# Leo-Liao-Chao/Uncertainty-Aware-CILQR-for-Trajectory-Optimization

Measured on AMD Instinct MI355X. Metric: CILQR solves/sec (N=50, batch B), higher is better.
Workload: dtype f64

## Files before the change

### uncertainty-aware-cilqr-for-trajectory-optimization_amd/csrc/cilqr_solve.hip

```cpp
#include <type_traits>

#include "cilqr_device.hpp"

namespace cilqr {

using namespace dev;

namespace {

constexpr int FREC = 16;

__device__ __forceinline__ double readfirstlane_f64(double v) {
  int lo = __double2loint(v), hi = __double2hiint(v);
  lo = __builtin_amdgcn_readfirstlane(lo);
  hi = __builtin_amdgcn_readfirstlane(hi);
  return __hiloint2double(hi, lo);
}

__device__ __forceinline__ double wave_sum(double v) {
#pragma unroll
  for (int o = 32; o > 0; o >>= 1) v += __shfl_xor(v, o, WAVE);
  return v;
}

// ... 414 lines not shown
  mfma_place(cur.AA, cur.sAA, slotA, low, cst);
  mfma_place(cur.BB, cur.sBB, slotB, low, cst);
  mfma_place(cur.Ca, cur.sCa, odd ? slotX : slotXX, low, cst);
  mfma_place(cur.Cb, cur.sCb, odd ? slotUU : C0, low, cst);
  double m00 = e == 0 ? 1.0 : 0.0, m01 = e == 1 || e == 4 ? 1.0 : 0.0, m11 = e == 5 ? 1.0 : 0.0;
  double mvc = odd && (lane & 3) == 2 ? 1.0 : 0.0;
  double lamb = lamb_in, lamb0 = lamb_in * (inv_half_dt * inv_half_dt);
  double lamb_row = (lane >> 4) == 0 ? lamb0 : lamb;
  CILQR_PIN(m00); CILQR_PIN(m01); CILQR_PIN(m11); CILQR_PIN(mvc); CILQR_PIN(lamb); CILQR_PIN(lamb0); CILQR_PIN(lamb_row);
  const bool stores = lane == 6 || lane == 22 || lane < 4 || (lane >= 16 && lane < 20);
  const int gslot = lane == 6 ? 0 : lane == 22 ? 1 : lane < 4 ? 2 + lane : 6 + (lane & 3);
  unsigned goff = stores ? (unsigned)(((N - 1) * FREC + gslot) * 8) : (unsigned)((N * FREC + (lane & 15)) * 8);
  const unsigned gstride = stores ? FREC * 8 : 0;
  char* const gbase = reinterpret_cast<char*>(fwd);
  double* gp = kK + (N - 1) * RECF + (stores ? gslot : 10 + (lane & 3));

  MfmaOperands oa, ob;
  cur.upper(oa);
  double V = odd_blocks_from_even(oa.Ca), vc = oa.Ca * mvc;
  int signs_v = 0, signs_s = 0;
  double det0 = 0.0;
  auto step = [&](const MfmaOperands& o) {
    unsigned long long s0 = 0, s1 = 0, s2 = 0, s3 = 0;
    if (DIAG) stamp_request(s0, V);
    const double P = CILQR_MFMA(V, o.AB, vc);
    const double Db = CILQR_MFMA(o.BB, P, o.Cb);
    const double Da = CILQR_MFMA(o.AA, P, o.Ca);
    const double a = readlane_f64(Db, 4), b = readlane_f64(Db, 5), d = readlane_f64(Db, 21);
    if (DIAG) stamp_request(s1, a + b + d);
    const double bb = b * b;
    det0 = fma(a, d, -bb);
    signs_v |= __double2hiint(det0);
    signs_s |= __double2hiint(a) | __double2hiint(d);
    const double ar = a + lamb0, dr = d + lamb;
    const double nr = -rcp_newton(fma(ar, dr, -bb));
    if (DIAG) stamp_request(s2, nr);
    const double adj = fma(ar, m11, fma(-b, m01, dr * m00));
    const double Dk = CILQR_MFMA(adj, Db, 0.0) * nr;
    const double H0 = fma(lamb_row, Dk, Db);
    const double H = odd_blocks_from_even(H0);
    double Dv = CILQR_MFMA(H, Dk, Da);
    vc = Dv * mvc;
    CILQR_PIN(vc);
    CILQR_PIN(Dv);
    V = odd_blocks_from_even(Dv);
    if (FSMEM) {
      *reinterpret_cast<double*>(gbase + goff) = Dk;
      goff -= gstride;
      asm volatile("" : "+v"(goff));
    } else {
      *gp = Dk;
      gp -= RECF;
    }
    if (DIAG) {
      stamp_request(s3, V);
      stamps_collect(s0, s1, s2, s3);
      sub[5] += s1 - s0; sub[6] += s2 - s1; sub[7] += s3 - s2;
    }
  };
  auto trip = [&] {
    cur.lower(ob);
    step(oa);
    cur.back();
    cur.upper(oa);
    step(ob);
  };
  bool two_left;
  if (FSMEM) {
    two_left = ((N - 1) & 1) != 0;
    for (int trips = (N - 1) >> 1; trips > 0; --trips) trip();
  } else {
    int j = N - 1;
    for (; j >= 2; j -= 2) trip();
    two_left = j == 1;
  }
  if (two_left) {
    cur.lower(ob);
    step(oa);
    step(ob);
  } else {
    step(oa);
  }
  return __builtin_amdgcn_ballot_w64((signs_v | signs_s) < 0 || !(det0 == det0)) == 0;
}

template <int KS>
__device__ __forceinline__ void load_fwd(FwdIn& o, const double* X, const double* U, const double* kK, int i) {
  const double* xo = X + i * XR;
  o.x = xo[0]; o.y = xo[1]; o.v = xo[2]; o.th = xo[3];
  o.u0 = U[2 * i]; o.u1 = U[2 * i + 1];
  const double* g = kK + i * KS;
#pragma unroll
  for (int k = 0; k < KR; ++k) o.g[k] = g[k];
}

__device__ __forceinline__ void fwd_step_store(const FwdConst& k, const FwdIn& c, State& s, double& max_turn, double inv_half_dt,
                                               double* Un_i, double* Xn_next) {
  double u0, u1;
  forward_step<true>(k, c, s, max_turn, u0, u1, inv_half_dt);
  Un_i[0] = u0; Un_i[1] = u1;
  Xn_next[0] = s.x; Xn_next[1] = s.y; Xn_next[2] = s.v; Xn_next[3] = s.th; Xn_next[4] = s.c; Xn_next[5] = s.s;
}

typedef double d2_t __attribute__((ext_vector_type(2)));
typedef __attribute__((address_space(3))) d2_t lds_d2;
constexpr int FSTEP = FREC * 8;
static_assert(XR % 2 == 0, "state records are whole 16-byte pairs");
struct FwdBump {
  unsigned& off;
  lds_d2*& un;
  lds_d2*& xn;
  template <int J> __device__ __forceinline__ void pin(double& ps, double& pc) const {
    if (J == 0) {
      asm volatile("" : "+v"(ps), "+v"(pc) : "v"(un));
      un += 2;
      asm volatile("" : "+v"(un));
    } else if (J == 1) {
      asm volatile("" : "+v"(ps), "+v"(pc) : "v"(xn));
      xn += XR;
      asm volatile("" : "+v"(xn));
    } else if (J == 2) {
      asm volatile("" : "+v"(ps), "+v"(pc) : "s"(off));
      off += 2 * FSTEP;
      asm volatile("" : "+s"(off));
    } else {
      CILQR_PIN2(ps, pc);
    }
  }
};
typedef double d8_t __attribute__((ext_vector_type(8)));
struct FwdS { d8_t lo, hi; };
__device__ __forceinline__ void f_sload_first(FwdS& r, const double* p) {
  asm volatile("s_load_dwordx16 %0, %2, 0x0\n\ts_load_dwordx16 %1, %2, 0x40" : "=&s"(r.lo), "=&s"(r.hi) : "s"(p) : "memory");
}
template <int AHEAD>
__device__ __forceinline__ void f_sload_next(FwdS& r, const double* fwd, unsigned off) {
  asm volatile("s_load_dwordx16 %0, %2, %3 offset:%4\n\ts_load_dwordx16 %1, %2, %3 offset:%5"
               : "+s"(r.lo), "+s"(r.hi) : "s"(fwd), "s"(off), "n"(AHEAD), "n"(AHEAD + 64) : "memory");
}
__device__ __forceinline__ void f_swait(FwdS& r) {
  __builtin_amdgcn_s_waitcnt(0xC07F);
  asm volatile("" : "+s"(r.lo), "+s"(r.hi) : : "memory");
}
__device__ __forceinline__ void f_sunpack(FwdIn& o, const FwdS& r) {
  o.g[0] = r.lo[0]; o.g[1] = r.lo[1]; o.g[2] = r.lo[2]; o.g[3] = r.lo[3]; o.g[4] = r.lo[4]; o.g[5] = r.lo[5];
  o.g[6] = r.lo[6]; o.g[7] = r.lo[7]; o.g[8] = r.hi[0]; o.g[9] = r.hi[1];
  o.x = r.hi[2]; o.y = r.hi[3]; o.v = r.hi[4]; o.th = r.hi[5]; o.u0 = r.hi[6]; o.u1 = r.hi[7];
}

template <bool PUBLISH = false>
__device__ __forceinline__ bool forward_smem(const KParams& kp, int N, const double* X, const double* fwd, double* Xn, double* Un) {
  asm volatile("s_waitcnt vmcnt(0)\n\ts_dcache_inv\n\ts_waitcnt lgkmcnt(0)" ::: "memory");
  FwdConst k;
  make_fwd_const(k, kp);
  double ihd = 2.0 / kp.dt;
  CILQR_PIN(ihd);
  State s;
  s.x = X[0]; s.y = X[1]; s.v = X[2]; s.th = X[3]; s.c = X[4]; s.s = X[5];
  store_state(Xn, 0, s);
  double max_turn = 0.0;
  FwdS r;
  FwdIn c;
  f_sload_first(r, fwd);
  unsigned off = 0;
  lds_d2* un = (lds_d2*)Un;
  lds_d2* xn = (lds_d2*)(Xn + XR);
// ... 149 lines not shown

  const double* wts = TAB != 2 ? obs_weights(a, b) : nullptr;
  if (TAB == 2) {
    sampled_prologue<WAVE>(a, kp, b, N, M, tab, off, rmax);
  } else if (!tab_shared) {
    const bool held = a.obs_ts == 0;
    for (int m = 0; m < M; ++m) {
      ObsEntry e;
      if (held) e = obs_entry_at(kp, a, b, m, 0);
      for (int t = lane; t < N; t += WAVE) {
        if (!held) e = obs_entry_at(kp, a, b, m, t);
        double* o = tab + ((size_t)m * N + t) * TABF;
        o[0] = e.ox; o[1] = e.oy; o[2] = e.co; o[3] = e.so; o[4] = e.ia2; o[5] = e.ib2;
      }
    }
  }
  __syncthreads();
  {
    double m = 0.0;
    for (int q = lane; q + 1 < S; q += WAVE) {
      const double d = fabs(samp[q + 1] - samp[q]);
      m = fmax(m, d == d ? d : __builtin_huge_val());
    }
    grid.dmax = wave_max_uniform(m);
  }

  UncPose upose{0, 0, 1, 0};
  if (has_unc) upose = unc_pose(a.unc, b);
  bool handover = false;
  if (GENERAL) {
    const double* x0 = a.x0 + (size_t)b * 4;
    State s;
    s.x = x0[0]; s.y = x0[1]; s.v = x0[2]; s.th = x0[3];
    sincos_fast(s.th, &s.s, &s.c);
    if (lane == 0) store_state(Xa, 0, s);
    for (int i = 0; i < N; ++i) {
      s = dyn_step(kp, s, Ua[2 * i], Ua[2 * i + 1]);
      if (lane == 0) store_state(Xa, i + 1, s);
    }
  } else {
    handover = !rollout_fast(kp, N, a.x0 + (size_t)b * 4, Ua, Xa) || (a.flags & CILQR_FLAG_GENERAL_ONLY) != 0;
  }
  __syncthreads();

  CILQR_STAMP(c_pro)
  double* Xc = Xa;
  double* Uc = Ua;
  double* Xn = Xb;
  double* Un = Ub;
  double J_old = DBL_MAX, lamb = 1.0, J_new = 0.0;
  int iters = 0, status = CILQR_EXIT_MAX_ITER, n_pass = 0;
  bool j_valid = false;
  const bool faithful = (a.flags & CILQR_FLAG_FAITHFUL_ITERS) != 0;
  const int max_it = kp.max_iterations;
  for (int it = 0; it < max_it && !handover; ++it) {
    ++iters;
    {
      double part;
      const KParams kpl = phase_params();
      const UncArgs* unc = has_unc ? &phase_args().unc : nullptr;
      if (TAB == 2) part = linearize<RECW, FSMEM, DIAG>(kpl, N, n_entries, lane, samp, S, grid, Xc, Uc, rec, SampledSource{tab, off, rmax, Xc, N, a.n_samples, M, a.samp_w, kpl.ego_front, kpl.ego_rear,
                                                     sqrt(1.0 + 64.0 / kpl.q2_front), sqrt(1.0 + 64.0 / kpl.q2_rear)}, unc, upose, b, fwd, sub);
      else part = linearize<RECW, FSMEM, DIAG>(kpl, N, n_entries, lane, samp, S, grid, Xc, Uc, rec, TabSource<TAB == 0>{tab, wts, N, kpl.w_obstacle}, unc, upose, b, fwd, sub);
      unsigned long long sub_t = 0;
      if (DIAG) sub_t = stamp_after(part);
      J_new = wave_sum_uniform(part);
      CILQR_SUB(4, J_new)
    }
    j_valid = true;
    __syncthreads();
    CILQR_STAMP(c_L)
    if (DIAG) ++n_L;
    const bool accept = J_new < J_old;
    if (!accept && !faithful) {
      if (J_new != J_new) { status = CILQR_EXIT_NUMERIC; break; }
      for (;;) {
        lamb = lamb * kp.lamb_factor;
        if (lamb > kp.lamb_max) { status = CILQR_EXIT_LAMBDA_MAX; break; }
        if (++it >= max_it) { status = CILQR_EXIT_MAX_ITER; break; }
        ++iters;
      }
      break;
    }
    if (!(GENERAL ? riccati<true>(kp, N, rec, kK, lamb) : riccati_mfma<FSMEM, DIAG>(N, rec, kK, fwd, cst, 2.0 / kp.dt, lamb, sub))) {
      if (GENERAL) { status = CILQR_EXIT_NUMERIC; break; }
      handover = true;
      break;
    }
    __syncthreads();
    CILQR_STAMP(c_R)
    ++n_pass;
    if (DIAG) ++n_R;
    if (GENERAL) {
      forward_general(kp, N, Xc, Uc, kK, Xn, Un);
    } else if (!(FSMEM ? forward_smem(KParams(phase_params()), N, Xc, fwd, Xn, Un) : forward_fast<RECW>(KParams(phase_params()), N, Xc, Uc, kK, Xn, Un))) {
      handover = true;
      break;
    }
    __syncthreads();
    CILQR_STAMP(c_F)
    if (accept) {
      double* t0 = Xc; Xc = Xn; Xn = t0;
      double* t1 = Uc; Uc = Un; Un = t1;
      j_valid = false;
      lamb = lamb / kp.lamb_factor;
      if (fabs(J_new - J_old) < kp.tolerance) { status = CILQR_EXIT_TOLERANCE; break; }
    } else {
      lamb = lamb * kp.lamb_factor;
      if (lamb > kp.lamb_max) { status = CILQR_EXIT_LAMBDA_MAX; break; }
    }
    J_old = J_new;
  }

  if (!GENERAL) {
    int32_t* const hint = phase_args().hint_passes;
    if (lane == 0) {
      phase_args().redo[b] = handover ? 1 : 0;
      if (handover && hint) hint[b] = 63;
    }
    if (handover) return;
  }

  __syncthreads();
  const SolveArgs ae = phase_args();
  double* Uo = ae.U + (size_t)b * 2 * N;
  for (int i = lane; i < 2 * N; i += WAVE) Uo[i] = Uc[i];
  double* Xg = ae.X_out + (size_t)b * 4 * (N + 1);
  for (int i = lane; i < 4 * (N + 1); i += WAVE) Xg[i] = Xc[(i >> 2) * XR + (i & 3)];
  if (ae.J_out) {
    if (!j_valid) J_new = wave_sum_uniform(cost_only(ae.kp, N, lane, samp, S, grid, Xc, Uc));
    if (lane == 0) ae.J_out[b] = J_new;
  }
  if (lane == 0) {
    if (ae.iters_out) ae.iters_out[b] = iters;
    if (ae.status_out) ae.status_out[b] = status;
    if (ae.passes) ae.passes[b] = n_pass;
    if (ae.hint_passes && !GENERAL) ae.hint_passes[b] = n_pass;
  }
  if (DIAG && lane == 0 && a.diag) {
    const unsigned long long now_ = __builtin_readcyclecounter();
    unsigned long long* o = a.diag + (size_t)b * DIAG_SLOTS;
    o[0] = c_pro; o[1] = c_L; o[2] = c_R; o[3] = c_F; o[4] = now_ - tk; o[5] = n_L; o[6] = n_R; o[7] = now_ - tk0;
    for (int q = 0; q < 8; ++q) o[8 + q] = sub[q];
  }
#undef CILQR_STAMP
}

constexpr unsigned long long THETA_PENDING = 0x7FF00000DEADBEEFull;
constexpr int PAIR_SPIN = 1 << 16;
constexpr int CMD_GO = 1, CMD_EXIT = 2;
constexpr int PAIR_LAST = 10;

template <int K>
__device__ __forceinline__ double quad_bcast(double v) {
  return dpp_f64<K * 0x55>(v);
}
template <int K>
__device__ __forceinline__ int quad_bcast_i(int v) { return __builtin_amdgcn_update_dpp(v, v, K * 0x55, 0xF, 0xF, false); }

template <bool LONG_NAP>
__device__ __forceinline__ bool state_arrived(const double* X, int k, int& budget) {
  const volatile unsigned long long* p = reinterpret_cast<const volatile unsigned long long*>(X + k * XR + 3);
  while (*p == THETA_PENDING) {
    if (--budget < 0) return false;
    if (LONG_NAP) __builtin_amdgcn_s_sleep(16); else __builtin_amdgcn_s_sleep(1);
  }
  asm volatile("" ::: "memory");
// ... 149 lines not shown
  double* Xa = samp + ((S + 1) & ~1);
  double* Ua = Xa + (N + 1) * XR;
  double* rec = Ua + 2 * N;
  double* cst = rec + N * RECF;
  double* tab = cst + RCST;
  double* Jt = tab + (size_t)M * TABF * N;
  double* ctl = Jt + ((N + 1) & ~1);
  double* fwd = a.fwd + (size_t)b * (N + 1) * FREC;
  int* const cmd = reinterpret_cast<int*>(ctl + 1);

  SampleGrid grid;
  make_sample_grid(grid, a.xplan_fl[2 * b], a.xplan_fl[2 * b + 1], S);
  {
    const double* pc = a.poly + (size_t)b * CILQR_POLY_COEFFS;
    for (int s = tid; s < S; s += 2 * WAVE) {
      double xs;
      sample_xy(grid, pc, s, xs, samp[s]);
    }
  }
  const double* Ug = a.U + (size_t)b * 2 * N;
  for (int i = tid; i < 2 * N; i += 2 * WAVE) Ua[i] = Ug[i];
  if (tid < 16 && (tid & 7) < 5) cst[(tid & 7) + (tid >> 3) * RECF] = (tid & 7) == 0 ? 0.0 : (tid & 7) == 1 ? 1.0 : (tid & 7) == 2 ? kp.dt : (tid & 7) == 3 ? kp.w_vel * 2 : 2.0;
  const double* wts = obs_weights(a, b);
  for (int m = wave; m < M; m += 2) {
    for (int t = lane; t < N; t += WAVE) {
      const ObsEntry e = obs_entry_at(kp, a, b, m, t);
      double* o = tab + ((size_t)m * N + t) * TABF;
      o[0] = e.ox; o[1] = e.oy; o[2] = e.co; o[3] = e.so; o[4] = e.ia2; o[5] = e.ib2;
    }
  }
  mark_pending(Xa, N, tid, 2 * WAVE);
  if (tid == 0) { cmd[0] = 0; cmd[1] = 0; }
  __syncthreads();

  if (wave != 0) {
    {
      double m = 0.0;
      for (int q = lane; q + 1 < S; q += WAVE) {
        const double d = fabs(samp[q + 1] - samp[q]);
        m = fmax(m, d == d ? d : __builtin_huge_val());
      }
      grid.dmax = wave_max_uniform(m);
    }
    unsigned long long dg[4] = {0, 0, 0, 0};
    for (;;) {
      linearize_quads<DIAG>(KParams(phase_params()), N, M, lane, samp, S, grid, Xa, Ua, rec, tab, wts, fwd, Jt, ctl, dg);
      __syncthreads();
      __syncthreads();
      if (*reinterpret_cast<volatile int*>(cmd) != CMD_GO) break;
    }
    if (DIAG && lane == 0 && a.diag) {
      unsigned long long* o = a.diag + (size_t)b * DIAG_SLOTS + 8;
      o[0] = dg[0]; o[1] = dg[1]; o[2] = dg[2]; o[3] = dg[3];
    }
    return;
  }

  bool handover = !rollout_fast<true>(kp, N, a.x0 + (size_t)b * 4, Ua, Xa) || (a.flags & CILQR_FLAG_GENERAL_ONLY) != 0;
  const int dbg = DIAG ? (int)((a.flags >> 8) & 3) : 0;
  if (dbg) __syncthreads();
  __syncthreads();
  CILQR_STAMP(c_pro)
  double J_old = DBL_MAX, lamb = 1.0, J_new = 0.0;
  int iters = 0, status = CILQR_EXIT_MAX_ITER, n_pass = 0;
  const int max_it = kp.max_iterations;
  for (int it = 0; it < max_it && !handover; ++it) {
    ++iters;
    if (reinterpret_cast<volatile int*>(cmd)[1] != 0) { handover = true; break; }
    J_new = *reinterpret_cast<volatile double*>(ctl);
    if (DIAG) ++n_L;
    const bool accept = J_new < J_old;
    if (!accept) {
      if (J_new != J_new) { status = CILQR_EXIT_NUMERIC; break; }
      for (;;) {
        lamb = lamb * kp.lamb_factor;
        if (lamb > kp.lamb_max) { status = CILQR_EXIT_LAMBDA_MAX; break; }
        if (++it >= max_it) { status = CILQR_EXIT_MAX_ITER; break; }
        ++iters;
      }
      break;
    }
    mark_pending(Xa, N, lane, WAVE);
    CILQR_STAMP(c_L)
    if (!riccati_mfma<true, DIAG>(N, rec, rec, fwd, cst, 2.0 / kp.dt, lamb, sub)) { handover = true; break; }
    if (lane == 0) *reinterpret_cast<volatile int*>(cmd) = CMD_GO;
    __syncthreads();
    CILQR_STAMP(c_R)
    ++n_pass;
    if (DIAG) ++n_R;
    const bool f_ok = forward_smem<true>(KParams(phase_params()), N, Xa, fwd, Xa, Ua);
    CILQR_STAMP(c_F)
    if (dbg) __syncthreads();
    __syncthreads();
    CILQR_STAMP(c_L)
    if (!f_ok) { handover = true; break; }
    lamb = lamb / kp.lamb_factor;
    if (fabs(J_new - J_old) < kp.tolerance) {
      status = CILQR_EXIT_TOLERANCE;
      J_new = *reinterpret_cast<volatile double*>(ctl);
      break;
    }
    J_old = J_new;
    if (it + 1 >= max_it) J_new = *reinterpret_cast<volatile double*>(ctl);
  }
  if (lane == 0) *reinterpret_cast<volatile int*>(cmd) = CMD_EXIT;
  __syncthreads();

  int32_t* const hint = phase_args().hint_passes;
  if (lane == 0) {
    phase_args().redo[b] = handover ? 1 : 0;
    if (handover && hint) hint[b] = 63;
  }
  if (handover) return;

  const SolveArgs ae = phase_args();
  double* Uo = ae.U + (size_t)b * 2 * N;
  for (int i = lane; i < 2 * N; i += WAVE) Uo[i] = Ua[i];
  double* Xg = ae.X_out + (size_t)b * 4 * (N + 1);
  for (int i = lane; i < 4 * (N + 1); i += WAVE) Xg[i] = Xa[(i >> 2) * XR + (i & 3)];
  if (lane == 0) {
    if (ae.J_out) ae.J_out[b] = J_new;
    if (ae.iters_out) ae.iters_out[b] = iters;
    if (ae.status_out) ae.status_out[b] = status;
    if (ae.passes) ae.passes[b] = n_pass;
    if (ae.hint_passes) ae.hint_passes[b] = n_pass;
  }
  if (DIAG && lane == 0 && a.diag) {
    const unsigned long long now_ = __builtin_readcyclecounter();
    unsigned long long* o = a.diag + (size_t)b * DIAG_SLOTS;
    o[0] = c_pro; o[1] = c_L; o[2] = c_R; o[3] = c_F; o[4] = now_ - tk; o[5] = n_L; o[6] = n_R; o[7] = now_ - tk0;
    for (int q = 4; q < 8; ++q) o[8 + q] = sub[q];
  }
#undef CILQR_STAMP
}

template <int W, bool DIAG, bool UNC = false>
__global__ __launch_bounds__(W * WAVE, 2) void cilqr_solve_split_kernel(SolveArgs a) {
  unsigned long long tk0 = 0, tk = 0, c_pro = 0, c_L = 0, c_R = 0, c_F = 0, n_L = 0, n_R = 0;
  if (DIAG) tk0 = tk = __builtin_readcyclecounter();
#define CILQR_STAMP(acc)                                 \
  if (DIAG) {                                            \
    const unsigned long long now_ = __builtin_readcyclecounter(); \
    acc += now_ - tk;                                    \
    tk = now_;                                           \
  }
  extern __shared__ __attribute__((aligned(16))) double lds[];
  if ((int)blockIdx.x >= a.B) return;
  const int b = __builtin_amdgcn_readfirstlane(a.order ? a.order[blockIdx.x] : (int)blockIdx.x);
  if (b >= a.B) return;
  const int tid = threadIdx.x, lane = tid & (WAVE - 1);
  const int wave = __builtin_amdgcn_readfirstlane(tid >> 6);
  const KParams kp = a.kp;
  const int N = a.N, M = a.M, S = kp.n_samples, NSMP = a.n_samples;
  double* samp = lds;
  double* Xa = samp + ((S + 1) & ~1);
  double* Ua = Xa + (N + 1) * XR;
  double* rec = Ua + 2 * N;
  double* cst = rec + N * RECF;
  double* off = cst + RCST;
  double* rmax = off + (size_t)M * NSMP * OFFF;
  double* part = rmax + 2 * M;
  double* umap = part + (size_t)(W - 1) * 5 * N;
  double* ctl = part + ((((W - 1) + (UNC ? 1 : 0)) * 5 * N + 1) & ~1);
  int* const cmd = reinterpret_cast<int*>(ctl);
  double* tab = a.obs_tab + (size_t)b * M * NOMF * N;

  SampleGrid grid;
// ... 334 lines not shown
  for (int it = 0; it < max_it && !handover; ++it) {
    ++iters;
    {
      const KParams kpl = phase_params();
      double dx[STEPS], dy[STEPS], lx2[STEPS], Jt = 0.0;
#pragma unroll
      for (int c2 = 0; c2 < STEPS; ++c2) {
        dx[c2] = 0.0; dy[c2] = 0.0; lx2[c2] = 0.0;
        const int t = lane + c2 * WAVE;
        if (t < N) {
          const double* xr = Xa + t * XR;
          const double px = xr[0], py = xr[1], v = xr[2];
          const double u0 = Ua[2 * t], u1 = Ua[2 * t + 1];
          double2* q = reinterpret_cast<double2*>(fwd + t * FREC + 10);
          q[0] = make_double2(px, py);
          q[1] = make_double2(v, xr[3]);
          q[2] = make_double2(u0, u1);
          const int cs = closest_sample(S, grid, px, py, LdsSamples{samp, grid.xf, grid.dxs});
          dx[c2] = px - fma(grid.dxs, (double)cs, grid.xf);
          dy[c2] = py - samp[cs];
          const double dv = v - kpl.desired_speed;
          lx2[c2] = (2 * kpl.w_vel) * dv;
          Jt += stage_cost(kpl, dx[c2], dy[c2], dv, u0, u1);
          if (W == 2) {
            Rec c;
            double a1, a2, a3, a4;
            ctrl_args(kpl, u0, u1, v, a1, a2, a3, a4);
            const double e1 = exp_fast(a1);
            const double e2 = exp_fast(a2);
            const double e3 = exp_fast(a3);
            const double e4 = exp_fast(a4);
            ctrl_terms(kpl, u0, u1, e1, e2, e3, e4, c);
            double* r = rec + t * RECF;
            const double ih = 2.0 / kpl.dt;
            r[6] = c.lu0 * ih; r[7] = c.lu1; r[8] = c.luu0 * (ih * ih); r[9] = c.luu1;
          }
        }
      }
      J_new = wave_sum_uniform(Jt);
      unsigned long long w0 = 0;
      if (DIAG) w0 = stamp_after(J_new);
      __syncthreads();
      if (DIAG) c_wait += __builtin_readcyclecounter() - w0;
#pragma unroll
      for (int c2 = 0; c2 < STEPS; ++c2) {
        const int t = lane + c2 * WAVE;
        if (t < N) {
          const double* q = part + (size_t)t * 5;
          StepSums s5{q[0], q[1], q[2], q[3], q[4]};
          if (W == 3 && !UNC) {
            const double* qo = q + (size_t)N * 5;
            s5.lx0 += qo[0]; s5.lx1 += qo[1]; s5.h00 += qo[2]; s5.h01 += qo[3]; s5.h11 += qo[4];
          }
          double* r = rec + t * RECF;
          double lx0, lx1, l00, l01, l11;
          state_terms(kpl, dx[c2], dy[c2], s5, lx0, lx1, l00, l01, l11);
          if (UNC) {
            const double* qu = umap + (size_t)t * 5;
            lx0 += qu[0]; lx1 += qu[1]; l00 += qu[2]; l01 += qu[3]; l11 += qu[4];
          }
          r[0] = lx0; r[1] = lx1; r[2] = lx2[c2]; r[3] = l00; r[4] = l01; r[5] = l11;
        }
      }
      j_valid = true;
    }
    CILQR_STAMP(c_L)
    if (DIAG) ++n_L;
    const bool accept = J_new < J_old;
    bool stop = false;
    if (!accept) {
      if (J_new != J_new) {
        status = CILQR_EXIT_NUMERIC;
      } else {
        for (;;) {
          lamb = lamb * kp.lamb_factor;
          if (lamb > kp.lamb_max) { status = CILQR_EXIT_LAMBDA_MAX; break; }
          if (++it >= max_it) { status = CILQR_EXIT_MAX_ITER; break; }
          ++iters;
        }
      }
      stop = true;
    } else {
      asm volatile("s_waitcnt lgkmcnt(0)" ::: "memory");
      if (!riccati_mfma<true, false>(N, rec, rec, fwd, cst, 2.0 / kp.dt, lamb, nullptr)) {
        handover = true;
        stop = true;
      } else {
        CILQR_STAMP(c_R)
        ++n_pass;
        if (DIAG) ++n_R;
        if (!forward_smem(KParams(phase_params()), N, Xa, fwd, Xa, Ua)) {
          handover = true;
          stop = true;
        } else {
          j_valid = false;
          lamb = lamb / kp.lamb_factor;
          if (fabs(J_new - J_old) < kp.tolerance) { status = CILQR_EXIT_TOLERANCE; stop = true; }
          J_old = J_new;
          if (it + 1 >= max_it) stop = true;
        }
      }
    }
    if (stop && lane == 0) *reinterpret_cast<volatile int*>(cmd) = CMD_EXIT;
    __syncthreads();
    CILQR_STAMP(c_F)
    if (stop) break;
  }

  int32_t* const hint = phase_args().hint_passes;
  if (lane == 0) {
    phase_args().redo[b] = handover ? 1 : 0;
    if (handover && hint) hint[b] = 63;
  }
  if (handover) return;

  const SolveArgs ae = phase_args();
  double* Uo = ae.U + (size_t)b * 2 * N;
  for (int i = lane; i < 2 * N; i += WAVE) Uo[i] = Ua[i];
  double* Xg = ae.X_out + (size_t)b * 4 * (N + 1);
  for (int i = lane; i < 4 * (N + 1); i += WAVE) Xg[i] = Xa[(i >> 2) * XR + (i & 3)];
  if (ae.J_out) {
    if (!j_valid) J_new = wave_sum_uniform(cost_only(ae.kp, N, lane, samp, S, grid, Xa, Ua));
    if (lane == 0) ae.J_out[b] = J_new;
  }
  if (lane == 0) {
    if (ae.iters_out) ae.iters_out[b] = iters;
    if (ae.status_out) ae.status_out[b] = status;
    if (ae.passes) ae.passes[b] = n_pass;
    if (ae.hint_passes) ae.hint_passes[b] = n_pass;
  }
  if (DIAG && lane == 0 && a.diag) {
    const unsigned long long now_ = __builtin_readcyclecounter();
    unsigned long long* o = a.diag + (size_t)b * DIAG_SLOTS;
    o[0] = c_pro; o[1] = c_L; o[2] = c_R; o[3] = c_F; o[4] = now_ - tk; o[5] = n_L; o[6] = n_R; o[7] = now_ - tk0;
    o[10] = c_wait;
    o[12] = (unsigned long long)__builtin_amdgcn_s_getreg((4) | (0 << 6) | (31 << 11)) |
            ((unsigned long long)__builtin_amdgcn_s_getreg((20) | (0 << 6) | (31 << 11)) << 32);
    if (W == 2) { o[11] = 0; o[14] = 0; }
    o[15] = 0;
  }
#undef CILQR_STAMP
}

__global__ void quu_inverse_kernel(int n, const double* q, const double* lamb, double* out, int general) {
  const int i = blockIdx.x * blockDim.x + threadIdx.x;
  if (i >= n) return;
  const double a = q[4 * i], b = 0.5 * (q[4 * i + 1] + q[4 * i + 2]), d = q[4 * i + 3];
  double i00 = 0, i01 = 0, i11 = 0;
  bool ok = true;
  if (general) ok = quu_inverse_general(a, b, d, lamb[i], i00, i01, i11);
  else quu_inverse_psd(a, b, d, lamb[i], b * b, i00, i01, i11);
  const double nan = __builtin_nan("");
  out[4 * i] = ok ? i00 : nan; out[4 * i + 1] = ok ? i01 : nan; out[4 * i + 2] = ok ? i01 : nan; out[4 * i + 3] = ok ? i11 : nan;
}

__global__ void closest_sample_kernel(int n, int S, const double* in, int32_t* out) {
  const int i = blockIdx.x * blockDim.x + threadIdx.x;
  if (i >= n) return;
  const double* q = in + (size_t)i * 10;
  double pc[CILQR_POLY_COEFFS];
  for (int j = 0; j < CILQR_POLY_COEFFS; ++j) pc[j] = q[j];
  SampleGrid g;
  make_sample_grid(g, q[6], q[7], S);
  auto at = [&](int s, double& x, double& y) { sample_xy(g, pc, s, x, y); };
  double m = 0.0, A = 0.0, B = 0.0, yp = 0.0;
  for (int s = 0; s < S; ++s) {
    double x, y, a2, a3;
// ... 130 lines not shown
```

Measured before the change: 2.498 million.

## Add LDS-addressed MFMA Riccati backward pass with deferred PSD check

Adds a specialized Riccati backward pass for the shared-memory path. It reads operands through explicit LDS address-space pointers with per-lane slot cursors. The positive-definiteness and NaN check is moved out of the serial recursion into a parallel post-pass over the stored Q blocks, which removes per-step sign tracking from the critical path. It also writes Q blocks back to LDS and gains into fwd inside the loop. Call sites in the FSMEM and persistent paths now use it, except the W==3 variant, trading more code and extra LDS writes for a shorter dependency chain.

```diff
diff --git a/uncertainty-aware-cilqr-for-trajectory-optimization_amd/csrc/cilqr_solve.hip b/uncertainty-aware-cilqr-for-trajectory-optimization_amd/csrc/cilqr_solve.hip
--- a/uncertainty-aware-cilqr-for-trajectory-optimization_amd/csrc/cilqr_solve.hip
+++ b/uncertainty-aware-cilqr-for-trajectory-optimization_amd/csrc/cilqr_solve.hip
@@ -520,6 +520,141 @@
     step(oa);
   }
   return __builtin_amdgcn_ballot_w64((signs_v | signs_s) < 0 || !(det0 == det0)) == 0;
+}
+
+typedef __attribute__((address_space(3))) double lds_f64;
+struct MfmaLdsCursor {
+  const lds_f64 *AB, *AA, *BB, *Ca, *Cb;
+  int sAB, sAA, sBB, sCa, sCb;
+  __device__ __forceinline__ void upper(MfmaOperands& o) const { o.AB = AB[RECF]; o.AA = AA[RECF]; o.BB = BB[RECF]; o.Ca = Ca[RECF]; o.Cb = Cb[RECF]; }
+  __device__ __forceinline__ void lower(MfmaOperands& o) const { o.AB = AB[0]; o.AA = AA[0]; o.BB = BB[0]; o.Ca = Ca[0]; o.Cb = Cb[0]; }
+};
+__device__ __forceinline__ void mfma_place(const lds_f64*& ptr, int& stride, int slot, const lds_f64* low, const lds_f64* cst) {
+  ptr = slot >= 0 ? low + slot : cst + (-1 - slot);
+  stride = slot >= 0 ? 2 * RECF : 0;
+}
+
+template <bool DIAG>
+__device__ __forceinline__ bool riccati_mfma_smem(int N, const double* rec, double* fwd, const double* cst, double inv_half_dt, double lamb_in,
+                                                  unsigned long long* sub) {
+  constexpr int C0 = -1, C1 = -2, CDT = -3, CW = -4, C2 = -5;
+  const int lane = threadIdx.x;
+  const int e = ((lane >> 4) << 2) | (lane & 3);
+  const bool odd = (lane & 4) != 0;
+  const int slotA = e == 0 || e == 5 || e == 10 || e == 15 ? C1 : e == 2 ? 10 : e == 6 ? 11 : e == 3 ? 12 : e == 7 ? 13 : C0;
+  const int slotB = e == 0 ? 10 : e == 4 ? 11 : e == 8 ? C2 : e == 13 ? CDT : C0;
+  const int slotXX = e == 0 ? 3 : e == 1 || e == 4 ? 4 : e == 5 ? 5 : e == 10 ? CW : C0;
+  const int slotX = e == 2 ? 0 : e == 6 ? 1 : e == 10 ? 2 : C0;
+  const int slotUU = e == 0 ? 8 : e == 5 ? 9 : e == 2 ? 6 : e == 6 ? 7 : C0;
+  using PTR = const lds_f64*;
+  const PTR low = (PTR)rec + (N - 2) * RECF;
+  const PTR cstp = (PTR)cst;
+  MfmaLdsCursor cur;
+  mfma_place(cur.AB, cur.sAB, odd ? slotB : slotA, low, cstp);
+  mfma_place(cur.AA, cur.sAA, slotA, low, cstp);
+  mfma_place(cur.BB, cur.sBB, slotB, low, cstp);
+  mfma_place(cur.Ca, cur.sCa, odd ? slotX : slotXX, low, cstp);
+  mfma_place(cur.Cb, cur.sCb, odd ? slotUU : C0, low, cstp);
+  double m00 = e == 0 ? 1.0 : 0.0, m01 = e == 1 || e == 4 ? 1.0 : 0.0, m11 = e == 5 ? 1.0 : 0.0;
+  double mvc = odd && (lane & 3) == 2 ? 1.0 : 0.0;
+  double lamb = lamb_in, lamb0 = lamb_in * (inv_half_dt * inv_half_dt);
+  double lamb_row = (lane >> 4) == 0 ? lamb0 : lamb;
+  CILQR_PIN(m00); CILQR_PIN(m01); CILQR_PIN(m11); CILQR_PIN(mvc); CILQR_PIN(lamb); CILQR_PIN(lamb0); CILQR_PIN(lamb_row);
+  const bool stores = lane == 6 || lane == 22 || lane < 4 || (lane >= 16 && lane < 20);
+  const int gslot = lane == 6 ? 0 : lane == 22 ? 1 : lane < 4 ? 2 + lane : 6 + (lane & 3);
+  unsigned goff = stores ? (unsigned)(((N - 1) * FREC + gslot) * 8) : (unsigned)((N * FREC + (lane & 15)) * 8);
+  const unsigned gstride = stores ? FREC * 8 : 0;
+  char* const gbase = reinterpret_cast<char*>(fwd);
+  lds_f64* qp = (lds_f64*)rec + (N - 2) * RECF + (lane == 4 ? 0 : lane == 5 ? 1 : lane == 21 ? 2 : 3 + lane % 11);
+
+  MfmaOperands oa, ob;
+  cur.upper(oa);
+  double V = odd_blocks_from_even(oa.Ca), vc = oa.Ca * mvc;
+  auto step = [&](const MfmaOperands& o, auto kind, auto upper_step) {
+    constexpr int KIND = decltype(kind)::value, QOFF = decltype(upper_step)::value ? RECF : 0;
+    unsigned long long s0 = 0, s1 = 0, s2 = 0, s3 = 0;
+    if (DIAG) stamp_request(s0, V);
+    const double P = CILQR_MFMA(V, o.AB, vc);
+    double Db = CILQR_MFMA(o.BB, P, o.Cb);
+    const double Da = CILQR_MFMA(o.AA, P, o.Ca);
+    if (KIND != 3) {
+      asm volatile("" : "+v"(Db) : "v"(cur.AB), "v"(cur.AA), "v"(cur.BB), "v"(cur.Ca), "v"(cur.Cb));
+      if (KIND == 1) cur.upper(oa); else cur.lower(ob);
+      asm volatile("");
+    }
+    const double a = readlane_f64(Db, 4), b = readlane_f64(Db, 5), d = readlane_f64(Db, 21);
+    if (DIAG) stamp_request(s1, a + b + d);
+    const double bb = b * b;
+    const double ar = a + lamb0, dr = d + lamb;
+    const double den = fma(ar, dr, -bb);
+    const double adj = fma(ar, m11, fma(-b, m01, dr * m00));
+    double Dkr = CILQR_MFMA(adj, Db, 0.0);
+    double r = __builtin_amdgcn_rcp(den);
+    asm volatile("" : "+v"(Dkr), "+v"(r), "+v"(goff) : "v"(qp));
+    qp[QOFF] = Db;
+    asm volatile("");
+    r = fma(fma(-den, r, 1.0), r, r);
+    r = fma(fma(-den, r, 1.0), r, r);
+    const double nr = -r;
+    if (DIAG) stamp_request(s2, nr);
+    const double Dk = Dkr * nr;
+    double H0 = fma(lamb_row, Dk, Db);
+    if (KIND == 0) {
+      asm volatile("" : "+v"(H0) : "v"(cur.AB), "v"(cur.AA));
+      cur.AB -= cur.sAB; cur.AA -= cur.sAA;
+    }
+    if (KIND == 1) {
+      asm volatile("" : "+v"(H0) : "v"(qp));
+      qp -= 2 * RECF;
+    }
+    double H = odd_blocks_from_even(H0);
+    if (KIND == 0) {
+      asm volatile("" : "+v"(H) : "v"(cur.BB), "v"(cur.Ca));
+      cur.BB -= cur.sBB; cur.Ca -= cur.sCa;
+    }
+    double Dv = CILQR_MFMA(H, Dk, Da);
+    asm volatile("" : "+v"(Dv) : "v"(goff));
+    *reinterpret_cast<double*>(gbase + goff) = Dk;
+    asm volatile("" : "+v"(Dv) : : "memory");
+    vc = Dv * mvc;
+    CILQR_PIN(vc);
+    asm volatile("" : "+v"(Dv) : "v"(goff), "v"(cur.Cb));
+    goff -= gstride;
+    if (KIND == 0) cur.Cb -= cur.sCb;
+    V = odd_blocks_from_even(Dv);
+    if (DIAG) {
+      stamp_request(s3, V);
+      stamps_collect(s0, s1, s2, s3);
+      sub[5] += s1 - s0; sub[6] += s2 - s1; sub[7] += s3 - s2;
+    }
+  };
+  using Upper = std::true_type;
+  using Lower = std::false_type;
+  using K0 = std::integral_constant<int, 0>;
+  using K1 = std::integral_constant<int, 1>;
+  using K2 = std::integral_constant<int, 2>;
+  using K3 = std::integral_constant<int, 3>;
+  for (int trips = (N - 1) >> 1; trips > 0; --trips) {
+    step(oa, K0(), Upper());
+    step(ob, K1(), Lower());
+  }
+  if (((N - 1) & 1) != 0) {
+    step(oa, K2(), Upper());
+    step(ob, K3(), Lower());
+  } else {
+    step(oa, K3(), Upper());
+  }
+  bool bad = false;
+  for (int base = 0; base < N; base += WAVE) {
+    const int t = base + lane;
+    const double* q = rec + (t < N ? t : N - 1) * RECF;
+    const double a = q[0], b = q[1], d = q[2];
+    const double bb = b * b;
+    const double det0 = fma(a, d, -bb);
+    const int signs = __double2hiint(det0) | __double2hiint(a) | __double2hiint(d);
+    bad |= t < N && (signs < 0 || (t == 0 && !(det0 == det0)));
+  }
+  return __builtin_amdgcn_ballot_w64(bad) == 0;
 }
 
 template <int KS>
@@ -835,7 +970,7 @@
       }
       break;
     }
-    if (!(GENERAL ? riccati<true>(kp, N, rec, kK, lamb) : riccati_mfma<FSMEM, DIAG>(N, rec, kK, fwd, cst, 2.0 / kp.dt, lamb, sub))) {
+    if (!(GENERAL ? riccati<true>(kp, N, rec, kK, lamb) : (FSMEM ? riccati_mfma_smem<DIAG>(N, rec, fwd, cst, 2.0 / kp.dt, lamb, sub) : riccati_mfma<false, DIAG>(N, rec, kK, fwd, cst, 2.0 / kp.dt, lamb, sub)))) {
       if (GENERAL) { status = CILQR_EXIT_NUMERIC; break; }
       handover = true;
       break;
@@ -1151,7 +1286,7 @@
     }
     mark_pending(Xa, N, lane, WAVE);
     CILQR_STAMP(c_L)
-    if (!riccati_mfma<true, DIAG>(N, rec, rec, fwd, cst, 2.0 / kp.dt, lamb, sub)) { handover = true; break; }
+    if (!riccati_mfma_smem<DIAG>(N, rec, fwd, cst, 2.0 / kp.dt, lamb, sub)) { handover = true; break; }
     if (lane == 0) *reinterpret_cast<volatile int*>(cmd) = CMD_GO;
     __syncthreads();
     CILQR_STAMP(c_R)
@@ -1652,7 +1787,8 @@
       stop = true;
     } else {
       asm volatile("s_waitcnt lgkmcnt(0)" ::: "memory");
-      if (!riccati_mfma<true, false>(N, rec, rec, fwd, cst, 2.0 / kp.dt, lamb, nullptr)) {
+      if (!(W == 3 ? riccati_mfma<true, false>(N, rec, rec, fwd, cst, 2.0 / kp.dt, lamb, nullptr)
+                   : riccati_mfma_smem<false>(N, rec, fwd, cst, 2.0 / kp.dt, lamb, nullptr))) {
         handover = true;
         stop = true;
       } else {
```

Result: faster. 2.539 million, median of 6 (+1.6%).
